# WJGiles/Dorknet

Measured on AMD Instinct MI355X. Metric: images/sec training step, ResNet-18-depsep 225x225 bs=256, 1/2/4/8 MI355X, higher is better.
Workload: dtype fp32; 1 GPU; ResNet-18-depsep 225x225 training step (fwd+loss+bwd+SGD-momentum), BASELINE config 3; global_batch=256, per_gpu_batch=256, parallelism=dp1, batch_norm=local

## Files before the change

dorknet_amd/csrc/pw_deep.hip:

```cpp
#include <stdlib.h>

#include <algorithm>
#include <atomic>

#include "dk_common.h"
#include "fold_tail.h"

#ifndef DK_PWD_EXP
#define DK_PWD_EXP 0
#endif

namespace dk {
namespace pwd {

constexpr int TR = 32;
constexpr int NW = 4;
constexpr int NB = 32 * NW;
constexpr int NT = 64 * NW;
typedef uint32_t u32x4 __attribute__((ext_vector_type(4)));
typedef uint32_t u32x2 __attribute__((ext_vector_type(2)));

template <int KR>
constexpr int fwd_wps() {
  return KR <= 64 ? 4 : KR <= 128 ? 3 : KR <= 256 ? 2 : 1;
}
template <int KR>
constexpr int dgrad_wps() {
  return KR <= 128 ? 2 : 1;
}

__device__ __forceinline__ uint32_t off4(int m, int ld, int c) { return ((uint32_t)m * ld + c) * 4u; }

__device__ __forceinline__ __amdgpu_buffer_rsrc_t tile_rsrc(const float* p, int ld, int tile, int nrows) {
  const int rows = nrows - tile * TR;
  return make_rsrc_v(p + (size_t)tile * TR * ld, rows > 0 ? (uint32_t)rows * ld * 4u : 0u);
}

constexpr int kAD = 4;

__device__ __forceinline__ int first_tile(int ntiles) {
  const int G = gridDim.x, r = ntiles % G, s = (r + 7) & ~7;
  return (int)((blockIdx.x + (unsigned)blockIdx.y * (unsigned)s) % (unsigned)G);
}
template <int KQ>
__device__ __forceinline__ void mfma_tile(const float* ap, const f32x4* bw, f32x16& acc) {
  constexpr int D = KQ < kAD ? KQ : kAD;
#pragma unroll
  for (int r = 0; r < 16; ++r) acc[r] = 0.f;
  f32x4 ab[D];
#pragma unroll
  for (int i = 0; i < D; ++i) ab[i] = ld4(ap + 8 * i);
#pragma unroll
  for (int q = 0; q < KQ; ++q) {
    const f32x4 av = ab[q % D];
    if (q + D < KQ) ab[q % D] = ld4(ap + 8 * (q + D));
    __builtin_amdgcn_sched_barrier(0);
#pragma unroll
    for (int e = 0; e < 4; ++e) acc = __builtin_amdgcn_mfma_f32_32x32x2f32(av[e], bw[q][e], acc, 0, 0, 0);
    __builtin_amdgcn_sched_barrier(0);
  }
}

__device__ __forceinline__ f32x4 cat4(f32x2 a, f32x2 b) { return f32x4{a[0], a[1], b[0], b[1]}; }
__device__ __forceinline__ f32x4 xhat4(f32x4 x, f32x4 m, f32x4 i) {
  return cat4((lo2(x) - lo2(m)) * lo2(i), (hi2(x) - hi2(m)) * hi2(i));
}
__device__ __forceinline__ f32x4 affine4(f32x4 xh, f32x4 g, f32x4 b) {
  return cat4(__builtin_elementwise_fma(lo2(g), lo2(xh), lo2(b)), __builtin_elementwise_fma(hi2(g), hi2(xh), hi2(b)));
}

struct FwdArgs {
  const float* x;
  const float* w;
  const float* bias;
  float* y;
  const float *im, *iis, *ig, *ib;
  int irelu;
  double* part;
  int M, N, H, W, OH, OW, sa;
  uint32_t xbytes;
  FoldTail ft;
  int nt;
};

__device__ __forceinline__ void partial_row(double ps, double pq, double* part, int N, int n0, const FoldTail& ft,
                                            float* scratch) {
  const int tid = threadIdx.x, lane = tid & 63, wave = tid >> 6, l32 = lane & 31, h = lane >> 5;
  double(*const red)[NB] = reinterpret_cast<double(*)[NB]>(scratch);
  ps += __shfl_xor(ps, 32, 64);
  pq += __shfl_xor(pq, 32, 64);
  __syncthreads();
  if (h == 0) {
    red[0][32 * wave + l32] = ps;
    red[1][32 * wave + l32] = pq;
  }
  __syncthreads();
  const int nc = N - n0 < NB ? N - n0 : NB;
  for (int i = tid; i < 2 * NB; i += NT) {
    const int which = i / NB, c = i - which * NB;
    if (c < nc) pub_store(part + ((size_t)blockIdx.x * 2 + which) * N + n0 + c, red[which][c]);
  }
  if (ft.part) {
    __syncthreads();
    fold_tail<NT>(ft, blockIdx.x, n0, nc, blockIdx.y, reinterpret_cast<double2*>(scratch));
  }
}

template <int KR, bool BN, bool STATS, bool STRIDED, bool HB>
__global__ __launch_bounds__(NT, fwd_wps<KR>()) void fwd_kernel(FwdArgs a) {
  constexpr int SK = KR + 4, KV = KR / 4, LV = TR * KV / NT, KQ = KR / 8;
  static_assert(KR % 32 == 0 && (SK / 4) % 2 == 1 && NT % KV == 0, "pwd::fwd_kernel shape");
  __shared__ __attribute__((aligned(16))) float As[2][TR * SK];
  static_assert(sizeof(double) * 2 * NT <= sizeof(float) * 2 * TR * SK, "fold scratch fits in the tiles");

  const int tid = threadIdx.x, lane = tid & 63, wave = tid >> 6;
  const int l32 = lane & 31, h = lane >> 5;
  const int n0 = blockIdx.y * NB, N = a.N;
  const int col = n0 + 32 * wave + l32;
  const float bias = HB ? a.bias[col] : 0.f;
  const bool irelu = a.irelu != 0;
  const int kv = tid % KV, r0 = tid / KV;
  f32x4 mu, is, ga, be;
  if constexpr (BN) {
    mu = ld4(a.im + 4 * kv);
    is = ld4(a.iis + 4 * kv);
    ga = ld4(a.ig + 4 * kv);
    be = ld4(a.ib + 4 * kv);
  }
  const __amdgpu_buffer_rsrc_t rx = make_rsrc_v(a.x, a.xbytes);
  const int ntiles = (a.M + TR - 1) / TR, G = gridDim.x;
  uint32_t lofs[LV], eofs[16];
#pragma unroll
  for (int j = 0; j < LV; ++j) lofs[j] = off4(r0 + j * (NT / KV), KR, 4 * kv);
#pragma unroll
  for (int r = 0; r < 16; ++r) eofs[r] = off4(4 * h + (r & 3) + 8 * (r >> 2), N, col);

  auto load_tile = [&](int tile, f32x4* st) {
    const __amdgpu_buffer_rsrc_t rt = tile_rsrc(a.x, KR, tile, a.M);
#pragma unroll
    for (int j = 0; j < LV; ++j) {
      if constexpr (STRIDED) {
        const int m = tile * TR + r0 + j * (NT / KV);
        const int ow = m % a.OW, q = m / a.OW, oh = q % a.OH, n = q / a.OH;
        const int row = (n * a.H + oh * a.sa) * a.W + ow * a.sa;
        st[j] = __builtin_bit_cast(f32x4, __builtin_amdgcn_raw_buffer_load_b128(rx, (int)off4(row, KR, 4 * kv), 0, 0));
      } else {
        st[j] = __builtin_bit_cast(f32x4, __builtin_amdgcn_raw_buffer_load_b128(rt, (int)lofs[j], 0, 0));
      }
    }
  };
  auto stage = [&](float* dst, const f32x4* st) {
    if (BN && irelu) {
#pragma unroll
      for (int j = 0; j < LV; ++j) {
        f32x4 v = st[j];
        if (!(DK_PWD_EXP & 2)) {
          v = affine4(xhat4(v, mu, is), ga, be);
#pragma unroll
          for (int e = 0; e < 4; ++e) v[e] = __builtin_fmaxf(v[e], 0.f);
        }
        st4(dst + (r0 + j * (NT / KV)) * SK + 4 * kv, v);
      }
    } else {
#pragma unroll
      for (int j = 0; j < LV; ++j) {
        f32x4 v = st[j];
        if constexpr (BN) v = affine4(xhat4(v, mu, is), ga, be);
        st4(dst + (r0 + j * (NT / KV)) * SK + 4 * kv, v);
      }
    }
  };

  int t = first_tile(ntiles);
  f32x4 bw[KQ];
  {
    f32x4 st[LV];
    load_tile(t, st);
#pragma unroll
    for (int q = 0; q < KQ; ++q)
      bw[q] = (DK_PWD_EXP & 8) ? f32x4{0.01f * q, 0.02f, 0.03f, (float)col} : ld4(a.w + (size_t)col * KR + 8 * q + 4 * h);
    stage(&As[0][0], st);
  }
  __syncthreads();
  double ps = 0.0, pq = 0.0;
  int buf = 0;
  for (; t < ntiles; t += G) {
    f32x4 nst[LV];
    load_tile(t + G, nst);
    const float* ap = &As[buf][0] + l32 * SK + 4 * h;
    f32x16 acc;
    mfma_tile<KQ>(ap, bw, acc);
    const int mb = t * TR + 4 * h;
    const __amdgpu_buffer_rsrc_t ry = tile_rsrc(a.y, N, t, a.M);
    if constexpr (HB) {
#pragma unroll
      for (int r = 0; r < 16; ++r) acc[r] += bias;
    }
#pragma unroll
    for (int r = 0; r < 16; ++r) {
      const float v = acc[r];
      if (!(DK_PWD_EXP & 1))
        bstore_nt(__builtin_bit_cast(uint32_t, v), ry, (int)eofs[r], 0, a.nt);
    }
    if constexpr (STATS) {
      if (t * TR + TR <= a.M) {
#pragma unroll
        for (int r = 0; r < 16; ++r) {
          const double d = (double)acc[r];
          ps += d;
          pq += d * d;
        }
      } else {
#pragma unroll
        for (int r = 0; r < 16; ++r) {
          const int dm = (r & 3) + 8 * (r >> 2);
          const double d = (mb + dm < a.M) ? (double)acc[r] : 0.0;
          ps += d;
          pq += d * d;
        }
      }
    }
    stage(&As[buf ^ 1][0], nst);
    __syncthreads();
    buf ^= 1;
  }
  if constexpr (STATS) partial_row(ps, pq, a.part, N, n0, a.ft, &As[0][0]);
}

struct DgradArgs {
  const float* g;
  const float* xo;
  float* dy_out;
  const float* w;
  float* dx;
  const float* res;
  const float* xi;
  const float *om, *ois, *og, *ob, *k12;
  int orelu;
  const float *im, *iis, *ig, *ib;
  int irelu;
  double* part;
  int M, N;
  FoldTail ft;
  int nt;
};

template <int KR, bool RES, bool PART, bool PLAIN = false>
__global__ __launch_bounds__(NT, dgrad_wps<KR>()) void dgrad_kernel(DgradArgs a) {
  constexpr int SK = KR + 4, KV = KR / 4, LV = TR * KV / NT, KQ = KR / 8;
  static_assert(KR % 32 == 0 && (SK / 4) % 2 == 1 && NT % KV == 0, "pwd::dgrad_kernel shape");
  __shared__ __attribute__((aligned(16))) float As[2][TR * SK];
  static_assert(sizeof(double) * 2 * NT <= sizeof(float) * 2 * TR * SK, "fold scratch fits in the tiles");

  const int tid = threadIdx.x, lane = tid & 63, wave = tid >> 6;
  const int l32 = lane & 31, h = lane >> 5;
  const int n0 = blockIdx.y * NB, N = a.N;
  const int col = n0 + 32 * wave + l32;
  const int kv = tid % KV, r0 = tid / KV;
  f32x4 mu = {}, is = {}, ga = {}, be = {}, k1 = {}, k2 = {}, f = {};
  if constexpr (!PLAIN) {
    mu = ld4(a.om + 4 * kv), is = ld4(a.ois + 4 * kv), ga = ld4(a.og + 4 * kv), be = ld4(a.ob + 4 * kv);
    k1 = ld4(a.k12 + 4 * kv), k2 = ld4(a.k12 + KR + 4 * kv);
#pragma unroll
    for (int e = 0; e < 4; ++e) f[e] = ga[e] * is[e];
  }
  const float pm = PART ? a.im[col] : 0.f, pis = PART ? a.iis[col] : 0.f, pga = PART ? a.ig[col] : 0.f,
              pbe = PART ? a.ib[col] : 0.f;
  const bool orelu = a.orelu != 0, irelu = a.irelu != 0;

  const bool writer = a.dy_out != nullptr && blockIdx.y == 0;
  const int ntiles = (a.M + TR - 1) / TR, G = gridDim.x;
  uint32_t lofs[LV], eofs[16];
#pragma unroll
  for (int j = 0; j < LV; ++j) lofs[j] = off4(r0 + j * (NT / KV), KR, 4 * kv);
#pragma unroll
  for (int r = 0; r < 16; ++r) eofs[r] = off4(4 * h + (r & 3) + 8 * (r >> 2), N, col);

  auto load_tile = [&](int tile, f32x4* sg, f32x4* sx) {
    const __amdgpu_buffer_rsrc_t rg = tile_rsrc(a.g, KR, tile, a.M), rx = tile_rsrc(a.xo, KR, tile, a.M);
#pragma unroll
    for (int j = 0; j < LV; ++j) {
      sg[j] = __builtin_bit_cast(f32x4, __builtin_amdgcn_raw_buffer_load_b128(rg, (int)lofs[j], 0, 0));
      if constexpr (!PLAIN)
        sx[j] = __builtin_bit_cast(f32x4, __builtin_amdgcn_raw_buffer_load_b128(rx, (int)lofs[j], 0, 0));
    }
  };
  auto stage = [&](int tile, float* dst, const f32x4* sg, const f32x4* sx) {
    const __amdgpu_buffer_rsrc_t rdy = tile_rsrc(writer ? a.dy_out : a.g, KR, tile, writer ? a.M : 0);
#pragma unroll
    for (int j = 0; j < LV; ++j) {
      const int r = r0 + j * (NT / KV);
      f32x4 v = sg[j];
      if constexpr (!PLAIN)
#pragma unroll
      for (int e = 0; e < 4; ++e) {
        const float xe = sx[j][e];
        float ge = sg[j][e];
        const bool kill = (!(bn_out(xe, mu[e], is[e], ga[e], be[e]) > 0.f)) & orelu;
        ge = kill ? 0.f : ge;
        v[e] = (DK_PWD_EXP & 2) ? ge + xe : bn_bwd_elem(xe, ge, mu[e], is[e], f[e], k1[e], k2[e]);
      }
      st4(dst + r * SK + 4 * kv, v);
      if constexpr (!PLAIN) bstore_nt(__builtin_bit_cast(u32x4, v), rdy, (int)lofs[j], 0, a.nt);
    }
  };

  int t = first_tile(ntiles);
  f32x4 bw[KQ];
  {
    f32x4 sg[LV], sx[LV];
    load_tile(t, sg, sx);
#pragma unroll
    for (int q = 0; q < KQ; ++q)
#pragma unroll
      for (int e = 0; e < 4; ++e) bw[q][e] = (DK_PWD_EXP & 8) ? 0.01f * q + e : a.w[(size_t)(8 * q + 4 * h + e) * N + col];
    stage(t, &As[0][0], sg, sx);
  }
  __syncthreads();
  double ps = 0.0, pq = 0.0;
  int buf = 0;
  for (; t < ntiles; t += G) {
    f32x4 ng[LV], nx[LV];
    load_tile(t + G, ng, nx);
    const int mb = t * TR + 4 * h;
    const __amdgpu_buffer_rsrc_t rxi = tile_rsrc(PART ? a.xi : a.g, N, t, PART ? a.M : 0);
    const __amdgpu_buffer_rsrc_t rr = tile_rsrc(RES ? a.res : a.g, N, t, RES ? a.M : 0);
    const __amdgpu_buffer_rsrc_t rdx = tile_rsrc(a.dx, N, t, a.M);
    float exi[16], ers[16];
#pragma unroll
    for (int r = 0; r < 16; ++r) {
      if constexpr (PART)
        exi[r] = __builtin_bit_cast(float, __builtin_amdgcn_raw_buffer_load_b32(rxi, (int)eofs[r], 0, 0));
      if constexpr (RES)
        ers[r] = __builtin_bit_cast(float, __builtin_amdgcn_raw_buffer_load_b32(rr, (int)eofs[r], 0, 0));
    }
    const float* ap = &As[buf][0] + l32 * SK + 4 * h;
    f32x16 acc;
    mfma_tile<KQ>(ap, bw, acc);
    if constexpr (RES) {
#pragma unroll
      for (int r = 0; r < 16; ++r) acc[r] += ers[r];
    }
#pragma unroll
    for (int r = 0; r < 16; ++r) {
      const float v = acc[r];
      if (!(DK_PWD_EXP & 1))
        bstore_nt(__builtin_bit_cast(uint32_t, v), rdx, (int)eofs[r], 0, a.nt);
    }
    if constexpr (PART) {
      const bool full = t * TR + TR <= a.M;
#pragma unroll
      for (int r = 0; r < 16; ++r) {
        const int dm = (r & 3) + 8 * (r >> 2);
        const float x = exi[r];
        const float xh = (x - pm) * pis;
        const bool kill = ((!(pga * xh + pbe > 0.f)) & irelu) | (!full && mb + dm >= a.M);
        const float gv = kill ? 0.f : acc[r];
        ps += (double)gv;
        pq += (double)gv * (double)xh;
      }
    }
    stage(t + G, &As[buf ^ 1][0], ng, nx);
    __syncthreads();
    buf ^= 1;
  }
  if constexpr (PART) partial_row(ps, pq, a.part, N, n0, a.ft, &As[0][0]);
}

constexpr int TR16 = 16;
constexpr int NW16 = 8;
constexpr int NT16 = 64 * NW16;

template <int KR>
struct K16 {
  static constexpr int RS = KR / 4 + 4;
  static constexpr int SK = 4 * RS + 4;
  static constexpr int KV = KR / 4;
  static constexpr int LV = TR16 * KV / NT16;
  static constexpr int NQ = KR / 16;
};

template <int NQ>
__device__ __forceinline__ void mfma16_tile(const float* ap, const f32x4* bw, f32x4& acc) {
  constexpr int D = 4;
  acc = f32x4{0.f, 0.f, 0.f, 0.f};
  f32x4 ab[D];
#pragma unroll
  for (int i = 0; i < D; ++i) ab[i] = ld4(ap + 4 * i);
#pragma unroll
  for (int q = 0; q < NQ; ++q) {
    const f32x4 av = ab[q % D];
    if (q + D < NQ) ab[q % D] = ld4(ap + 4 * (q + D));
    __builtin_amdgcn_sched_barrier(0);
#pragma unroll
    for (int u = 0; u < 4; ++u) acc = __builtin_amdgcn_mfma_f32_16x16x4f32(av[u], bw[q][u], acc, 0, 0, 0);
    __builtin_amdgcn_sched_barrier(0);
  }
}

template <int KR, bool RES, bool PART, bool PLAIN = false>
__global__ __launch_bounds__(NT16, 2) void dgrad16_kernel(DgradArgs a) {
  using L = K16<KR>;
  constexpr int SK = L::SK, RS = L::RS, KV = L::KV, LV = L::LV, NQ = L::NQ;
  static_assert(KR % 256 == 0 && (SK / 4) % 2 == 1 && NT16 % KV == 0 && LV >= 1, "pwd::dgrad16_kernel shape");
  __shared__ __attribute__((aligned(16))) float As[2][TR16 * SK];
  __shared__ __attribute__((aligned(16))) f32x4 bnt[7][KV];
  static_assert(sizeof(double) * 2 * NT16 <= sizeof(float) * 2 * TR16 * SK, "fold scratch fits in the tiles");

  const int tid = threadIdx.x, lane = tid & 63, wave = tid >> 6;
  const int c16 = lane & 15, kg = lane >> 4;
  const int n0 = blockIdx.y * NB, N = a.N;
  const int col = n0 + 16 * wave + c16;
  const int kvl = tid % KV, r0 = tid / KV;
  const int kv = (kvl & ~63) | ((kvl & 31) << 1) | ((kvl >> 5) & 1);
  if (!PLAIN && tid < KV) {
    const f32x4 ga = ld4(a.og + 4 * tid), is = ld4(a.ois + 4 * tid);
    bnt[0][tid] = ld4(a.om + 4 * tid);
    bnt[1][tid] = is;
    bnt[2][tid] = ga;
    bnt[3][tid] = ld4(a.ob + 4 * tid);
    bnt[4][tid] = ld4(a.k12 + 4 * tid);
    bnt[5][tid] = ld4(a.k12 + KR + 4 * tid);
    f32x4 f;
#pragma unroll
    for (int e = 0; e < 4; ++e) f[e] = ga[e] * is[e];
    bnt[6][tid] = f;
  }
  const float pm = PART ? a.im[col] : 0.f, pis = PART ? a.iis[col] : 0.f, pga = PART ? a.ig[col] : 0.f,
              pbe = PART ? a.ib[col] : 0.f;
  const bool orelu = a.orelu != 0, irelu = a.irelu != 0;
  const bool writer = a.dy_out != nullptr && blockIdx.y == 0;
  const int ntiles = (a.M + TR16 - 1) / TR16, G = gridDim.x;
  uint32_t lofs[LV];
#pragma unroll
  for (int j = 0; j < LV; ++j) lofs[j] = off4(r0 + j * (NT16 / KV), KR, 4 * kv);
  const uint32_t cbase = off4(4 * kg, N, col);
  const int sreg = (kv & 1) * RS + (kv & ~1);

  auto tile_rsrc16 = [&](const float* p, int ld, int tile, int nrows) {
    const int rows = nrows - tile * TR16;
    return make_rsrc_v(p + (size_t)tile * TR16 * ld, rows > 0 ? (uint32_t)rows * ld * 4u : 0u);
  };
  auto load_tile = [&](int tile, f32x4* sg, f32x4* sx) {
    const __amdgpu_buffer_rsrc_t rg = tile_rsrc16(a.g, KR, tile, a.M), rx = tile_rsrc16(a.xo, KR, tile, a.M);
#pragma unroll
    for (int j = 0; j < LV; ++j) {
      sg[j] = __builtin_bit_cast(f32x4, __builtin_amdgcn_raw_buffer_load_b128(rg, (int)lofs[j], 0, 0));
      if constexpr (!PLAIN)
        sx[j] = __builtin_bit_cast(f32x4, __builtin_amdgcn_raw_buffer_load_b128(rx, (int)lofs[j], 0, 0));
    }
  };
  auto stage = [&](int tile, float* dst, const f32x4* sg, const f32x4* sx) {
    const __amdgpu_buffer_rsrc_t rdy = tile_rsrc16(writer ? a.dy_out : a.g, KR, tile, writer ? a.M : 0);
#pragma unroll
    for (int j = 0; j < LV; ++j) {
      const int r = r0 + j * (NT16 / KV);
      f32x4 v = sg[j];
      if constexpr (!PLAIN) {
        const f32x4 mu = bnt[0][kv], is = bnt[1][kv], ga = bnt[2][kv], be = bnt[3][kv], k1 = bnt[4][kv],
                    k2 = bnt[5][kv], f = bnt[6][kv];
#pragma unroll
        for (int e = 0; e < 4; ++e) {
          const float xe = sx[j][e];
          float ge = sg[j][e];
          const bool kill = (!(bn_out(xe, mu[e], is[e], ga[e], be[e]) > 0.f)) & orelu;
          ge = kill ? 0.f : ge;
          v[e] = bn_bwd_elem(xe, ge, mu[e], is[e], f[e], k1[e], k2[e]);
        }
      }
      float* d = dst + r * SK + sreg;
      *reinterpret_cast<f32x2*>(d) = f32x2{v[0], v[2]};
      *reinterpret_cast<f32x2*>(d + 2 * RS) = f32x2{v[1], v[3]};
      if constexpr (!PLAIN) bstore_nt(__builtin_bit_cast(u32x4, v), rdy, (int)lofs[j], 0, a.nt);
    }
  };

  __syncthreads();
  int t = first_tile(ntiles);
  f32x4 bw[NQ];
  {
    f32x4 sg[LV], sx[LV];
    load_tile(t, sg, sx);
#pragma unroll
    for (int q = 0; q < NQ; ++q)
#pragma unroll
      for (int u = 0; u < 4; ++u) {
        const int i = 4 * q + u;
        const int k = 8 * (i >> 1) + 2 * (i & 1) + (kg >> 1) + 4 * (kg & 1);
        bw[q][u] = a.w[(size_t)k * N + col];
      }
    stage(t, &As[0][0], sg, sx);
  }
  __syncthreads();
  double ps = 0.0, pq = 0.0;
  int buf = 0;
  for (; t < ntiles; t += G) {
    f32x4 ng[LV], nx[LV];
    load_tile(t + G, ng, nx);
    const int mb = t * TR16 + 4 * kg;
    const __amdgpu_buffer_rsrc_t rxi = tile_rsrc16(PART ? a.xi : a.g, N, t, PART ? a.M : 0);
    const __amdgpu_buffer_rsrc_t rr = tile_rsrc16(RES ? a.res : a.g, N, t, RES ? a.M : 0);
    const __amdgpu_buffer_rsrc_t rdx = tile_rsrc16(a.dx, N, t, a.M);
    float exi[4], ers[4];
#pragma unroll
    for (int r = 0; r < 4; ++r) {
      if constexpr (PART)
        exi[r] = __builtin_bit_cast(float, __builtin_amdgcn_raw_buffer_load_b32(rxi, (int)cbase, r * N * 4, 0));
      if constexpr (RES)
        ers[r] = __builtin_bit_cast(float, __builtin_amdgcn_raw_buffer_load_b32(rr, (int)cbase, r * N * 4, 0));
    }
    f32x4 acc;
    mfma16_tile<NQ>(&As[buf][0] + c16 * SK + kg * RS, bw, acc);
    if constexpr (RES) {
#pragma unroll
      for (int r = 0; r < 4; ++r) acc[r] += ers[r];
    }
#pragma unroll
    for (int r = 0; r < 4; ++r) {
      const float v = acc[r];
      bstore_nt(__builtin_bit_cast(uint32_t, v), rdx, (int)cbase, r * N * 4, a.nt);
    }
    if constexpr (PART) {
      const bool full = t * TR16 + TR16 <= a.M;
#pragma unroll
      for (int r = 0; r < 4; ++r) {
        const float x = exi[r];
        const float xh = (x - pm) * pis;
        const bool kill = ((!(pga * xh + pbe > 0.f)) & irelu) | (!full && mb + r >= a.M);
        const float gv = kill ? 0.f : acc[r];
        ps += (double)gv;
        pq += (double)gv * (double)xh;
      }
    }
    stage(t + G, &As[buf ^ 1][0], ng, nx);
    __syncthreads();
    buf ^= 1;
  }
  if constexpr (PART) {
    double(*const red)[NB] = reinterpret_cast<double(*)[NB]>(&As[0][0]);
    ps += __shfl_xor(ps, 16, 64);
    pq += __shfl_xor(pq, 16, 64);
    ps += __shfl_xor(ps, 32, 64);
    pq += __shfl_xor(pq, 32, 64);
    __syncthreads();
    if (kg == 0) {
      red[0][16 * wave + c16] = ps;
      red[1][16 * wave + c16] = pq;
    }
    __syncthreads();
    for (int i = tid; i < 2 * NB; i += NT16) {
      const int which = i / NB, c = i - which * NB;
      pub_store(a.part + ((size_t)blockIdx.x * 2 + which) * N + n0 + c, red[which][c]);
    }
    if (a.ft.part) {
      __syncthreads();
      fold_tail<NT16>(a.ft, blockIdx.x, n0, NB, blockIdx.y, reinterpret_cast<double2*>(&As[0][0]));
    }
  }
}

struct BwdArgs {
  const float* g;
  const float* xo;
  const float* w;
  float* dx;
  const float* res;
  const float* xi;
  const float *om, *ois, *og, *ob, *k12;
  int orelu;
  const float *im, *iis, *ig, *ib;
  int irelu;
  double* part;
  float* wpart;
  int M, N;
  FoldTail ft;
  int nt;
};

template <int KR>
constexpr int bwd_wps() {
  return KR <= 128 ? 2 : 1;
}

template <int KR, bool RES, bool BNIN>
__global__ __launch_bounds__(NT, bwd_wps<KR>()) void bwd_kernel(BwdArgs a) {
  constexpr int SK = KR + 4, KV = KR / 4, LV = TR * KV / NT, KQ = KR / 8, NKT = KR / 32, NU = KR / 128;
  static_assert(KR % 128 == 0 && (SK / 4) % 2 == 1 && NT % KV == 0, "pwd::bwd_kernel shape");
  __shared__ __attribute__((aligned(16))) float As[2][TR * SK];
  __shared__ __attribute__((aligned(16))) f32x4 bnt[7][KV];
  static_assert(sizeof(double) * 2 * NT <= sizeof(float) * 2 * TR * SK, "fold scratch fits in the tiles");
  static_assert(32 * (NB + 4) <= 2 * TR * SK, "dW transpose tile fits in the tiles");

  const int tid = threadIdx.x, lane = tid & 63, wave = tid >> 6;
  const int l32 = lane & 31, h = lane >> 5;
  const int n0 = blockIdx.y * NB, N = a.N;
  const int col = n0 + 32 * wave + l32;
  const bool wact = n0 + 32 * wave < N;
  const int kv = tid % KV, r0 = tid / KV;
  if (tid < KV) {
    const f32x4 ga = ld4(a.og + 4 * tid), is = ld4(a.ois + 4 * tid);
    bnt[0][tid] = ld4(a.om + 4 * tid);
    bnt[1][tid] = is;
    bnt[2][tid] = ga;
    bnt[3][tid] = ld4(a.ob + 4 * tid);
    bnt[4][tid] = ld4(a.k12 + 4 * tid);
    bnt[5][tid] = ld4(a.k12 + KR + 4 * tid);
    f32x4 f;
#pragma unroll
    for (int e = 0; e < 4; ++e) f[e] = ga[e] * is[e];
    bnt[6][tid] = f;
  }
  __syncthreads();
  const float pm = BNIN && wact ? a.im[col] : 0.f, pis = BNIN && wact ? a.iis[col] : 0.f,
              pga = BNIN && wact ? a.ig[col] : 0.f, pbe = BNIN && wact ? a.ib[col] : 0.f;
  const bool orelu = a.orelu != 0, irelu = a.irelu != 0;

  const int ntiles = (a.M + TR - 1) / TR, G = gridDim.x;
  uint32_t lofs[LV];
#pragma unroll
  for (int j = 0; j < LV; ++j) lofs[j] = off4(r0 + j * (NT / KV), KR, 4 * kv);
  const uint32_t cbase = off4(4 * h, N, col);

  auto load_tile = [&](int tile, f32x4* sg, f32x4* sx) {
    const __amdgpu_buffer_rsrc_t rg = tile_rsrc(a.g, KR, tile, a.M), rx = tile_rsrc(a.xo, KR, tile, a.M);
#pragma unroll
    for (int j = 0; j < LV; ++j) {
      sg[j] = __builtin_bit_cast(f32x4, __builtin_amdgcn_raw_buffer_load_b128(rg, (int)lofs[j], 0, 0));
      sx[j] = __builtin_bit_cast(f32x4, __builtin_amdgcn_raw_buffer_load_b128(rx, (int)lofs[j], 0, 0));
    }
  };
  auto stage = [&](float* dst, const f32x4* sg, const f32x4* sx) {
    const f32x4 mu = bnt[0][kv], is = bnt[1][kv], ga = bnt[2][kv], be = bnt[3][kv], k1 = bnt[4][kv], k2 = bnt[5][kv],
                f = bnt[6][kv];
#pragma unroll
    for (int j = 0; j < LV; ++j) {
      const int r = r0 + j * (NT / KV);
      f32x4 v;
#pragma unroll
      for (int e = 0; e < 4; ++e) {
        const float xe = sx[j][e];
        float ge = sg[j][e];
        const bool kill = (!(bn_out(xe, mu[e], is[e], ga[e], be[e]) > 0.f)) & orelu;
        ge = kill ? 0.f : ge;
        v[e] = bn_bwd_elem(xe, ge, mu[e], is[e], f[e], k1[e], k2[e]);
      }
      st4(dst + r * SK + 4 * kv, v);
    }
  };

  int t = first_tile(ntiles);
  f32x4 bw[KQ];
  {
    f32x4 sg[LV], sx[LV];
    load_tile(t, sg, sx);
#pragma unroll
    for (int q = 0; q < KQ; ++q)
#pragma unroll
      for (int e = 0; e < 4; ++e) bw[q][e] = wact ? a.w[(size_t)(8 * q + 4 * h + e) * N + col] : 0.f;
    stage(&As[0][0], sg, sx);
  }
  __syncthreads();
  f32x16 dw[NKT];
#pragma unroll
  for (int i = 0; i < NKT; ++i)
#pragma unroll
    for (int r = 0; r < 16; ++r) dw[i][r] = 0.f;
  double ps = 0.0, pq = 0.0;
  int buf = 0;
  for (; t < ntiles; t += G) {
    f32x4 ng[LV], nx[LV];
    load_tile(t + G, ng, nx);
    const float* tile = &As[buf][0];
    if (wact) {
    const int mb = t * TR + 4 * h;
    const __amdgpu_buffer_rsrc_t rxi = tile_rsrc(a.xi, N, t, a.M);
    const __amdgpu_buffer_rsrc_t rr = tile_rsrc(RES ? a.res : a.xi, N, t, RES ? a.M : 0);
    const __amdgpu_buffer_rsrc_t rdx = tile_rsrc(a.dx, N, t, a.M);
    float ex[16], ers[16];
#pragma unroll
    for (int r = 0; r < 16; ++r) {
      const int ro = ((r & 3) + 8 * (r >> 2)) * N * 4;
      ex[r] = __builtin_bit_cast(float, __builtin_amdgcn_raw_buffer_load_b32(rxi, (int)cbase, ro, 0));
      if constexpr (RES) ers[r] = __builtin_bit_cast(float, __builtin_amdgcn_raw_buffer_load_b32(rr, (int)cbase, ro, 0));
    }
    f32x16 acc;
    mfma_tile<KQ>(tile + l32 * SK + 4 * h, bw, acc);
    if constexpr (RES) {
#pragma unroll
      for (int r = 0; r < 16; ++r) acc[r] += ers[r];
    }
#pragma unroll
    for (int r = 0; r < 16; ++r) {
      const float v = acc[r];
      bstore_nt(__builtin_bit_cast(uint32_t, v), rdx, (int)cbase, ((r & 3) + 8 * (r >> 2)) * N * 4, a.nt);
    }
    const bool full = t * TR + TR <= a.M;
    float yb[16];
#pragma unroll
    for (int r = 0; r < 16; ++r) {
      const int dm = (r & 3) + 8 * (r >> 2);
      const bool out = !full && mb + dm >= a.M;
      const float x = ex[r];
      if constexpr (BNIN) {
        const float xh = (x - pm) * pis;
        const float v = __builtin_fmaf(pga, xh, pbe);
        const bool dead = !(v > 0.f) & irelu;
        const float gv = (dead | out) ? 0.f : acc[r];
        ps += (double)gv;
        pq += (double)gv * (double)xh;
        yb[r] = (dead | out) ? 0.f : v;
      } else {
        yb[r] = out ? 0.f : x;
      }
    }
    {
      const float* bp = tile + (4 * h) * SK + 4 * l32;
      f32x4 bv[NU], nb[NU];
#pragma unroll
      for (int u = 0; u < NU; ++u) bv[u] = ld4(bp + 128 * u);
#pragma unroll
      for (int s = 0; s < 16; ++s) {
        if (s + 1 < 16) {
          const int pn = ((s + 1) & 3) + 8 * ((s + 1) >> 2);
#pragma unroll
          for (int u = 0; u < NU; ++u) nb[u] = ld4(bp + pn * SK + 128 * u);
        }
        __builtin_amdgcn_sched_barrier(0);
#pragma unroll
        for (int u = 0; u < NU; ++u)
#pragma unroll
          for (int e = 0; e < 4; ++e) dw[4 * u + e] = __builtin_amdgcn_mfma_f32_32x32x2f32(yb[s], bv[u][e], dw[4 * u + e], 0, 0, 0);
        __builtin_amdgcn_sched_barrier(0);
#pragma unroll
        for (int u = 0; u < NU; ++u) bv[u] = nb[u];
      }
    }
    }
    stage(&As[buf ^ 1][0], ng, nx);
    __syncthreads();
    buf ^= 1;
  }
  {
    constexpr int ST = NB + 4;
    float* T = &As[0][0];
    float* wp = a.wpart + (size_t)blockIdx.x * KR * N + n0;
#pragma unroll
    for (int kt = 0; kt < NKT; ++kt) {
      __syncthreads();
#pragma unroll
      for (int r = 0; r < 16; ++r) T[l32 * ST + 32 * wave + 4 * h + (r & 3) + 8 * (r >> 2)] = dw[kt][r];
      __syncthreads();
#pragma unroll
      for (int j = 0; j < 32 * NB / 4 / NT; ++j) {
        const int idx = tid + NT * j, i = idx / (NB / 4), c4 = idx % (NB / 4);
        const int k = 4 * i + (kt & 3) + 128 * (kt >> 2);
        if (n0 + 4 * c4 < N) st4(wp + (size_t)k * N + 4 * c4, ld4(T + i * ST + 4 * c4));
      }
    }
  }
  if constexpr (BNIN) partial_row(ps, pq, a.part, N, n0, a.ft, &As[0][0]);
}

template <int KR, bool RES, bool BNIN>
__global__ __launch_bounds__(NT16, 2) void bwd16_kernel(BwdArgs a) {
  using L = K16<KR>;
  constexpr int SK = L::SK, RS = L::RS, KV = L::KV, LV = L::LV, NQ = L::NQ, NKT = KR / 16;
  static_assert(KR % 256 == 0 && (SK / 4) % 2 == 1 && NT16 % KV == 0 && LV >= 1, "pwd::bwd16_kernel shape");
  __shared__ __attribute__((aligned(16))) float As[2][TR16 * SK];
  __shared__ __attribute__((aligned(16))) f32x4 bnt[7][KV];
  static_assert(sizeof(double) * 2 * NT16 <= sizeof(float) * 2 * TR16 * SK, "fold scratch fits in the tiles");

  const int tid = threadIdx.x, lane = tid & 63, wave = tid >> 6;
  const int c16 = lane & 15, kg = lane >> 4;
  const int n0 = blockIdx.y * NB, N = a.N;
  const int col = n0 + 16 * wave + c16;
  const int kvl = tid % KV, r0 = tid / KV;
  const int kv = (kvl & ~63) | ((kvl & 31) << 1) | ((kvl >> 5) & 1);
  if (tid < KV) {
    const f32x4 ga = ld4(a.og + 4 * tid), is = ld4(a.ois + 4 * tid);
    bnt[0][tid] = ld4(a.om + 4 * tid);
    bnt[1][tid] = is;
    bnt[2][tid] = ga;
    bnt[3][tid] = ld4(a.ob + 4 * tid);
    bnt[4][tid] = ld4(a.k12 + 4 * tid);
    bnt[5][tid] = ld4(a.k12 + KR + 4 * tid);
    f32x4 f;
#pragma unroll
    for (int e = 0; e < 4; ++e) f[e] = ga[e] * is[e];
    bnt[6][tid] = f;
  }
  const float pm = BNIN ? a.im[col] : 0.f, pis = BNIN ? a.iis[col] : 0.f, pga = BNIN ? a.ig[col] : 0.f,
              pbe = BNIN ? a.ib[col] : 0.f;
  const bool orelu = a.orelu != 0, irelu = a.irelu != 0;
  const int ntiles = (a.M + TR16 - 1) / TR16, G = gridDim.x;
  uint32_t lofs[LV];
#pragma unroll
  for (int j = 0; j < LV; ++j) lofs[j] = off4(r0 + j * (NT16 / KV), KR, 4 * kv);
  const uint32_t cbase = off4(4 * kg, N, col);
  const int sreg = (kv & 1) * RS + (kv & ~1);
  const int r8 = c16 & 7;
  const int doff = ((((r8 & 1) << 1) | ((r8 >> 2) & 1)) * RS) + 2 * (c16 >> 3) + ((r8 >> 1) & 1);

  auto tile_rsrc16 = [&](const float* p, int ld, int tile, int nrows) {
    const int rows = nrows - tile * TR16;
    return make_rsrc_v(p + (size_t)tile * TR16 * ld, rows > 0 ? (uint32_t)rows * ld * 4u : 0u);
  };
  auto load_tile = [&](int tile, f32x4* sg, f32x4* sx) {
    const __amdgpu_buffer_rsrc_t rg = tile_rsrc16(a.g, KR, tile, a.M), rx = tile_rsrc16(a.xo, KR, tile, a.M);
#pragma unroll
    for (int j = 0; j < LV; ++j) {
      sg[j] = __builtin_bit_cast(f32x4, __builtin_amdgcn_raw_buffer_load_b128(rg, (int)lofs[j], 0, 0));
      sx[j] = __builtin_bit_cast(f32x4, __builtin_amdgcn_raw_buffer_load_b128(rx, (int)lofs[j], 0, 0));
    }
  };
  auto stage = [&](float* dst, const f32x4* sg, const f32x4* sx) {
    const f32x4 mu = bnt[0][kv], is = bnt[1][kv], ga = bnt[2][kv], be = bnt[3][kv], k1 = bnt[4][kv], k2 = bnt[5][kv],
                f = bnt[6][kv];
#pragma unroll
    for (int j = 0; j < LV; ++j) {
      const int r = r0 + j * (NT16 / KV);
      f32x4 v;
#pragma unroll
      for (int e = 0; e < 4; ++e) {
        const float xe = sx[j][e];
        float ge = sg[j][e];
        const bool kill = (!(bn_out(xe, mu[e], is[e], ga[e], be[e]) > 0.f)) & orelu;
        ge = kill ? 0.f : ge;
        v[e] = bn_bwd_elem(xe, ge, mu[e], is[e], f[e], k1[e], k2[e]);
      }
      float* d = dst + r * SK + sreg;
      *reinterpret_cast<f32x2*>(d) = f32x2{v[0], v[2]};
      *reinterpret_cast<f32x2*>(d + 2 * RS) = f32x2{v[1], v[3]};
    }
  };

  __syncthreads();
  int t = first_tile(ntiles);
  f32x4 bw[NQ];
  {
    f32x4 sg[LV], sx[LV];
    load_tile(t, sg, sx);
#pragma unroll
    for (int q = 0; q < NQ; ++q)
#pragma unroll
      for (int u = 0; u < 4; ++u) {
        const int i = 4 * q + u;
        const int k = 8 * (i >> 1) + 2 * (i & 1) + (kg >> 1) + 4 * (kg & 1);
        bw[q][u] = a.w[(size_t)k * N + col];
      }
    stage(&As[0][0], sg, sx);
  }
  __syncthreads();
  f32x4 dw[NKT];
#pragma unroll
  for (int i = 0; i < NKT; ++i) dw[i] = f32x4{0.f, 0.f, 0.f, 0.f};
  double ps = 0.0, pq = 0.0;
  int buf = 0;
  for (; t < ntiles; t += G) {
    f32x4 ng[LV], nx[LV];
    load_tile(t + G, ng, nx);
    const int mb = t * TR16 + 4 * kg;
    const __amdgpu_buffer_rsrc_t rxi = tile_rsrc16(a.xi, N, t, a.M);
    const __amdgpu_buffer_rsrc_t rr = tile_rsrc16(RES ? a.res : a.xi, N, t, RES ? a.M : 0);
    const __amdgpu_buffer_rsrc_t rdx = tile_rsrc16(a.dx, N, t, a.M);
    float ex[4], ers[4];
#pragma unroll
    for (int r = 0; r < 4; ++r) {
      ex[r] = __builtin_bit_cast(float, __builtin_amdgcn_raw_buffer_load_b32(rxi, (int)cbase, r * N * 4, 0));
      if constexpr (RES)
        ers[r] = __builtin_bit_cast(float, __builtin_amdgcn_raw_buffer_load_b32(rr, (int)cbase, r * N * 4, 0));
    }
    const float* tile = &As[buf][0];
    f32x4 acc;
    mfma16_tile<NQ>(tile + c16 * SK + kg * RS, bw, acc);
    if constexpr (RES) {
#pragma unroll
      for (int r = 0; r < 4; ++r) acc[r] += ers[r];
    }
#pragma unroll
    for (int r = 0; r < 4; ++r) {
      const float v = acc[r];
      bstore_nt(__builtin_bit_cast(uint32_t, v), rdx, (int)cbase, r * N * 4, a.nt);
    }
    const bool full = t * TR16 + TR16 <= a.M;
    float yb[4];
#pragma unroll
    for (int r = 0; r < 4; ++r) {
      const bool out = !full && mb + r >= a.M;
      const float x = ex[r];
      if constexpr (BNIN) {
        const float xh = (x - pm) * pis;
        const float v = __builtin_fmaf(pga, xh, pbe);
        const bool dead = !(v > 0.f) & irelu;
        const float gv = (dead | out) ? 0.f : acc[r];
        ps += (double)gv;
        pq += (double)gv * (double)xh;
        yb[r] = (dead | out) ? 0.f : v;
      } else {
        yb[r] = out ? 0.f : x;
      }
    }
    {
      const float* bp = tile + (4 * kg) * SK + doff;
#pragma unroll
      for (int r = 0; r < 4; ++r) {
        float bv[NKT];
#pragma unroll
        for (int kt = 0; kt < NKT; ++kt) bv[kt] = bp[r * SK + 4 * kt];
#pragma unroll
        for (int kt = 0; kt < NKT; ++kt) dw[kt] = __builtin_amdgcn_mfma_f32_16x16x4f32(yb[r], bv[kt], dw[kt], 0, 0, 0);
      }
    }
    stage(&As[buf ^ 1][0], ng, nx);
    __syncthreads();
    buf ^= 1;
  }
  {
    float* wp = a.wpart + (size_t)blockIdx.x * KR * N + n0 + 16 * wave + 4 * kg;
#pragma unroll
    for (int kt = 0; kt < NKT; ++kt) st4(wp + (size_t)(16 * kt + c16) * N, dw[kt]);
  }
  if constexpr (BNIN) {
    double(*const red)[NB] = reinterpret_cast<double(*)[NB]>(&As[0][0]);
    ps += __shfl_xor(ps, 16, 64);
    pq += __shfl_xor(pq, 16, 64);
    ps += __shfl_xor(ps, 32, 64);
    pq += __shfl_xor(pq, 32, 64);
    __syncthreads();
    if (kg == 0) {
      red[0][16 * wave + c16] = ps;
      red[1][16 * wave + c16] = pq;
    }
    __syncthreads();
    for (int i = tid; i < 2 * NB; i += NT16) {
      const int which = i / NB, c = i - which * NB;
      pub_store(a.part + ((size_t)blockIdx.x * 2 + which) * N + n0 + c, red[which][c]);
    }
    if (a.ft.part) {
      __syncthreads();
      fold_tail<NT16>(a.ft, blockIdx.x, n0, NB, blockIdx.y, reinterpret_cast<double2*>(&As[0][0]));
    }
  }
}

#define DK_PWD_KR(X) X(64) X(128) X(256) X(512)
#define DK_PWD_KR_DGRAD(X) X(64) X(128) X(256)

static int occupancy(const void* fn, int nt = NT) {
  int v = 0;
  if (hipOccupancyMaxActiveBlocksPerMultiprocessor(&v, fn, nt, 0) != hipSuccess || v < 1) v = 1;
  return v;
}

template <int KR>
static int fwd_occ() {
  static const int occ = [] {
#define DK_F(B_, S_, T_) reinterpret_cast<const void*>(&fwd_kernel<KR, B_, S_, T_, false>), \
                         reinterpret_cast<const void*>(&fwd_kernel<KR, B_, S_, T_, true>)
    const void* fs[] = {DK_F(true, true, false), DK_F(true, false, false), DK_F(false, true, false),
                        DK_F(false, false, false), DK_F(true, true, true), DK_F(true, false, true),
                        DK_F(false, true, true), DK_F(false, false, true)};
#undef DK_F
    int o = 1 << 20;
    for (const void* f : fs) o = std::min(o, occupancy(f));
    return o;
  }();
  return occ;
}
template <int KR>
static int dgrad_occ() {
  static const int occ = [] {
    const void* fs[] = {reinterpret_cast<const void*>(&dgrad_kernel<KR, true, true>),
                        reinterpret_cast<const void*>(&dgrad_kernel<KR, true, false>),
                        reinterpret_cast<const void*>(&dgrad_kernel<KR, false, true>),
                        reinterpret_cast<const void*>(&dgrad_kernel<KR, false, false>)};
    int o = 1 << 20;
    for (const void* f : fs) o = std::min(o, occupancy(f));
    return o;
  }();
  return occ;
}

template <int KR>
static int dgrad16_occ() {
  static const int occ = [] {
    const void* fs[] = {reinterpret_cast<const void*>(&dgrad16_kernel<KR, true, true>),
                        reinterpret_cast<const void*>(&dgrad16_kernel<KR, true, false>),
                        reinterpret_cast<const void*>(&dgrad16_kernel<KR, false, true>),
                        reinterpret_cast<const void*>(&dgrad16_kernel<KR, false, false>)};
    int o = 1 << 20;
    for (const void* f : fs) o = std::min(o, occupancy(f, NT16));
    return o;
  }();
  return occ;
}

template <int KR>
static int bwd16_occ() {
  static const int occ = [] {
    const void* fs[] = {reinterpret_cast<const void*>(&bwd16_kernel<KR, true, true>),
                        reinterpret_cast<const void*>(&bwd16_kernel<KR, true, false>),
                        reinterpret_cast<const void*>(&bwd16_kernel<KR, false, true>),
                        reinterpret_cast<const void*>(&bwd16_kernel<KR, false, false>)};
    int o = 1 << 20;
    for (const void* f : fs) o = std::min(o, occupancy(f, NT16));
    return o;
  }();
  return occ;
}

template <int KR>
static int bwd_occ() {
  static const int occ = [] {
    const void* fs[] = {reinterpret_cast<const void*>(&bwd_kernel<KR, true, true>),
                        reinterpret_cast<const void*>(&bwd_kernel<KR, true, false>),
                        reinterpret_cast<const void*>(&bwd_kernel<KR, false, true>),
                        reinterpret_cast<const void*>(&bwd_kernel<KR, false, false>)};
    int o = 1 << 20;
    for (const void* f : fs) o = std::min(o, occupancy(f));
    return o;
  }();
  return occ;
}

static int grid_x(int M, int N, int occ, int tr = TR) {
  const int ntiles = (M + tr - 1) / tr;
  const int groups = N < NB ? 1 : N / NB;
  int slots = occ * 256 / groups;
  if (slots < 1) slots = 1;
  int gx = std::min(ntiles, slots);
  const int g8 = gx / 8 * 8;
  if (g8 >= 8 && (ntiles + g8 - 1) / g8 == (ntiles + gx - 1) / gx) gx = g8;
  return gx;
}

}

static bool pwd_enabled() { return knob(kKnobPwDeep) == 1 && pw_stream_enabled(); }

static bool pwd_kr(int KR) { return KR == 64 || KR == 128 || KR == 256 || KR == 512; }

bool pw_deep_fwd_ok(int K, int C, int M, size_t xbytes) {
  if (!pwd_enabled() || M <= 0 || (K < 128 && C < 128) || !pwd_kr(C) || K % pwd::NB) return false;
  return xbytes < ((size_t)1 << 31) && (size_t)M * K * 4 < ((size_t)1 << 31);
}
bool pw_deep_dgrad_ok(int K, int C, int M) {
  if (!pwd_enabled() || M <= 0 || (K < 128 && C < 128) || !pwd_kr(K) || C % pwd::NB) return false;
  return (size_t)M * (K > C ? K : C) * 4 < ((size_t)1 << 31);
}

int pw_deep_fwd_rows(int M, int K, int C) {
#define DK_ROWS(kr) \
  if (C == kr) return pwd::grid_x(M, K, pwd::fwd_occ<kr>());
  DK_PWD_KR(DK_ROWS)
#undef DK_ROWS
  return 0;
}
int pw_deep_fwd_slices(int M, int K, int C) { return K / pwd::NB; }
static bool pwd_dgrad16(int K) { return K == 512; }

int pw_deep_dgrad_rows(int M, int K, int C) {
  if (pwd_dgrad16(K)) return pwd::grid_x(M, C, pwd::dgrad16_occ<512>(), pwd::TR16);
#define DK_ROWS(kr) \
  if (K == kr) return pwd::grid_x(M, C, pwd::dgrad_occ<kr>());
  DK_PWD_KR_DGRAD(DK_ROWS)
#undef DK_ROWS
  return 0;
}
int pw_deep_dgrad_slices(int M, int K, int C) { return C / pwd::NB; }

int pw_deep_fwd(const float* x, int N, int H, int W, int stride, int OH, int OW, const float* w, int K, int C,
                const float* bias, float* y, const float* im, const float* iis, const float* ig, const float* ib,
                int irelu, double* part, hipStream_t st, const FoldTail* ft) {
  const int M = N * OH * OW;
  const bool strided = stride != 1 || H != OH || W != OW;
  pwd::FwdArgs a{x, w, bias, y, im, iis, ig, ib, irelu, part, M, K, H, W, OH, OW, stride,
                 (uint32_t)((size_t)N * H * W * C * 4)};
  if (ft && part) a.ft = *ft;
  a.nt = nt_stores(kNtPwd);
  const dim3 grid(pw_deep_fwd_rows(M, K, C), K / pwd::NB);
  if (grid.x == 0) return DK_ERR_ARGS;
#define DK_L(kr, B_, S_, T_)                                                                          \
  do {                                                                                                \
    if (bias)                                                                                         \
      hipLaunchKernelGGL((pwd::fwd_kernel<kr, B_, S_, T_, true>), grid, dim3(pwd::NT), 0, st, a);     \
    else                                                                                              \
      hipLaunchKernelGGL((pwd::fwd_kernel<kr, B_, S_, T_, false>), grid, dim3(pwd::NT), 0, st, a);    \
  } while (0)
#define DK_FWD(kr)                    \
  if (C == kr) {                      \
    if (strided) {                    \
      if (im && part)                 \
        DK_L(kr, true, true, true);   \
      else if (im)                    \
        DK_L(kr, true, false, true);  \
      else if (part)                  \
        DK_L(kr, false, true, true);  \
      else                            \
        DK_L(kr, false, false, true); \
    } else if (im && part)            \
      DK_L(kr, true, true, false);    \
    else if (im)                      \
      DK_L(kr, true, false, false);   \
    else if (part)                    \
      DK_L(kr, false, true, false);   \
    else                              \
      DK_L(kr, false, false, false);  \
    return launch_status();           \
  }
  DK_PWD_KR(DK_FWD)
#undef DK_FWD
#undef DK_L
  return DK_ERR_ARGS;
}

int pw_deep_dgrad_bnbwd(const float* g, const float* bn_x, int M, int K, int C, const float* om, const float* ois,
                        const float* og, const float* ob, int orelu, const float* k12, float* dy_out, const float* w,
                        float* dx, const float* res, const float* x, const float* im, const float* iis,
                        const float* ig, const float* ib, int irelu, double* part, hipStream_t st,
                        const FoldTail* ft) {
  pwd::DgradArgs a{g, bn_x, dy_out, w, dx, res, x, om, ois, og, ob, k12, orelu, im, iis, ig, ib, irelu, part, M, C};
  if (ft && part) a.ft = *ft;
  a.nt = nt_stores(kNtPwd);
  const dim3 grid(pw_deep_dgrad_rows(M, K, C), C / pwd::NB);
  if (grid.x == 0) return DK_ERR_ARGS;
  if (pwd_dgrad16(K)) {
#define DK_L16(R_, P_) hipLaunchKernelGGL((pwd::dgrad16_kernel<512, R_, P_>), grid, dim3(pwd::NT16), 0, st, a)
    if (res && x)
      DK_L16(true, true);
    else if (res)
      DK_L16(true, false);
    else if (x)
      DK_L16(false, true);
    else
      DK_L16(false, false);
#undef DK_L16
    return launch_status();
  }
#define DK_L(kr, R_, P_) hipLaunchKernelGGL((pwd::dgrad_kernel<kr, R_, P_>), grid, dim3(pwd::NT), 0, st, a)
#define DK_DG(kr)             \
  if (K == kr) {              \
    if (res && x)             \
      DK_L(kr, true, true);   \
    else if (res)             \
      DK_L(kr, true, false);  \
    else if (x)               \
      DK_L(kr, false, true);  \
    else                      \
      DK_L(kr, false, false); \
    return launch_status();   \
  }
  DK_PWD_KR_DGRAD(DK_DG)
#undef DK_DG
#undef DK_L
  return DK_ERR_ARGS;
}

int pw_deep_dgrad_plain(const float* dy, int M, int K, int C, const float* w, float* dx, hipStream_t st) {
  pwd::DgradArgs a{dy, nullptr, nullptr, w, dx, nullptr, nullptr, nullptr, nullptr, nullptr, nullptr, nullptr, 0,
                   nullptr, nullptr, nullptr, nullptr, 0, nullptr, M, C};
  a.nt = nt_stores(kNtPwd);
  const dim3 grid(pw_deep_dgrad_rows(M, K, C), C / pwd::NB);
  if (grid.x == 0) return DK_ERR_ARGS;
  if (pwd_dgrad16(K)) {
    hipLaunchKernelGGL((pwd::dgrad16_kernel<512, false, false, true>), grid, dim3(pwd::NT16), 0, st, a);
    return launch_status();
  }
#define DK_DG(kr)                                                                                           \
  if (K == kr) {                                                                                            \
    hipLaunchKernelGGL((pwd::dgrad_kernel<kr, false, false, true>), grid, dim3(pwd::NT), 0, st, a);         \
    return launch_status();                                                                                 \
  }
  DK_PWD_KR_DGRAD(DK_DG)
#undef DK_DG
  return DK_ERR_ARGS;
}

static bool pwd_bwd_enabled() { return knob(kKnobPwDeepBwd) == 1 && pwd_enabled(); }
bool pw_deep_bwd_ok(int K, int C, int M) {
  if (!pwd_bwd_enabled() || M <= 0 || (K != 128 && K != 256) || (C % pwd::NB && !(K == 128 && C == 64)))
    return false;
  return (size_t)M * (K > C ? K : C) * 4 < ((size_t)1 << 31);
}
static bool pwd_bwd16(int K) { return K == 256; }

int pw_deep_bwd_rows(int M, int K, int C) {
  if (pwd_bwd16(K)) return pwd::grid_x(M, C, pwd::bwd16_occ<256>(), pwd::TR16);
  if (K == 128) return pwd::grid_x(M, C, pwd::bwd_occ<128>());
  return 0;
}
int pw_deep_bwd_slices(int M, int K, int C) { return C < pwd::NB ? 1 : C / pwd::NB; }

int pw_deep_bwd_bnbwd(const float* g, const float* bn_x, int M, int K, int C, const float* om, const float* ois,
                      const float* og, const float* ob, int orelu, const float* k12, const float* w, float* dx,
                      const float* res, const float* x, const float* im, const float* iis, const float* ig,
                      const float* ib, int irelu, double* part, float* wpart, hipStream_t st, const FoldTail* ft) {
  if ((im != nullptr) != (part != nullptr)) return DK_ERR_ARGS;
  pwd::BwdArgs a{g, bn_x, w, dx, res, x, om, ois, og, ob, k12, orelu, im, iis, ig, ib, irelu, part, wpart, M, C};
  if (ft && part) a.ft = *ft;
  a.nt = nt_stores(kNtPwd);
  const dim3 grid(pw_deep_bwd_rows(M, K, C), pw_deep_bwd_slices(M, K, C));
  if (grid.x == 0) return DK_ERR_ARGS;
  if (pwd_bwd16(K)) {
#define DK_L16(kr, R_, B_) hipLaunchKernelGGL((pwd::bwd16_kernel<kr, R_, B_>), grid, dim3(pwd::NT16), 0, st, a)
#define DK_B16(kr)             \
  if (K == kr) {               \
    if (res && im)             \
      DK_L16(kr, true, true);  \
    else if (res)              \
      DK_L16(kr, true, false); \
    else if (im)               \
      DK_L16(kr, false, true); \
    else                       \
      DK_L16(kr, false, false); \
    return launch_status();    \
  }
    DK_B16(256)
#undef DK_B16
#undef DK_L16
  }
#define DK_L(kr, R_, B_) hipLaunchKernelGGL((pwd::bwd_kernel<kr, R_, B_>), grid, dim3(pwd::NT), 0, st, a)
#define DK_BW(kr)             \
  if (K == kr) {              \
    if (res && im)            \
      DK_L(kr, true, true);   \
    else if (res)             \
      DK_L(kr, true, false);  \
    else if (im)              \
      DK_L(kr, false, true);  \
    else                      \
      DK_L(kr, false, false); \
    return launch_status();   \
  }
  DK_BW(128)
#undef DK_BW
#undef DK_L
  return DK_ERR_ARGS;
}


}
```

Measured before the change: 33310 images/s.

## Add specialized pointwise backward kernel for K=128, C=64 processing tile pairs

Adds a dedicated fused backward kernel for the K=128, C=64 pointwise layer. The generic kernel uses a 128-column block, which leaves half of it idle when C is 64. The new kernel has each pair of waves cover the 64 columns and work on one of two 32-row tiles, so each block handles 64 rows per step. The two waves' dW partials are summed through shared memory before they are written. This is meant to recover the lanes wasted on the narrow layer, at the cost of more code, extra register pressure and an extra shared-memory reduction pass.

```diff
diff --git a/dorknet_amd/csrc/pw_deep.hip b/dorknet_amd/csrc/pw_deep.hip
--- a/dorknet_amd/csrc/pw_deep.hip
+++ b/dorknet_amd/csrc/pw_deep.hip
@@ -761,6 +761,207 @@
   if constexpr (BNIN) partial_row(ps, pq, a.part, N, n0, a.ft, &As[0][0]);
 }
 
+constexpr int TP = 2 * TR;
+
+template <bool RES, bool BNIN>
+__global__ __launch_bounds__(NT, 2) void bwd64_kernel(BwdArgs a) {
+  constexpr int KR = 128, N = 64, SK = KR + 4, KV = KR / 4, LV = TR * KV / NT, KQ = KR / 8, NKT = KR / 32;
+  static_assert((SK / 4) % 2 == 1 && NT % KV == 0, "pwd::bwd64_kernel shape");
+  __shared__ __attribute__((aligned(16))) float As[2][TP * SK];
+  __shared__ __attribute__((aligned(16))) f32x4 bnt[7][KV];
+  static_assert(sizeof(double) * 2 * NT <= sizeof(float) * 2 * TP * SK, "fold scratch fits in the tiles");
+  static_assert(32 * (N + 4) <= 2 * TP * SK, "dW transpose tile fits in the tiles");
+
+  const int tid = threadIdx.x, lane = tid & 63, wave = tid >> 6;
+  const int l32 = lane & 31, h = lane >> 5;
+  const int wp = __builtin_amdgcn_readfirstlane(wave >> 1);
+  const int col = 32 * (wave & 1) + l32;
+  const int kv = tid % KV, r0 = tid / KV;
+  if (tid < KV) {
+    const f32x4 ga = ld4(a.og + 4 * tid), is = ld4(a.ois + 4 * tid);
+    bnt[0][tid] = ld4(a.om + 4 * tid);
+    bnt[1][tid] = is;
+    bnt[2][tid] = ga;
+    bnt[3][tid] = ld4(a.ob + 4 * tid);
+    bnt[4][tid] = ld4(a.k12 + 4 * tid);
+    bnt[5][tid] = ld4(a.k12 + KR + 4 * tid);
+    f32x4 f;
+#pragma unroll
+    for (int e = 0; e < 4; ++e) f[e] = ga[e] * is[e];
+    bnt[6][tid] = f;
+  }
+  __syncthreads();
+  const float pm = BNIN ? a.im[col] : 0.f, pis = BNIN ? a.iis[col] : 0.f, pga = BNIN ? a.ig[col] : 0.f,
+              pbe = BNIN ? a.ib[col] : 0.f;
+  const bool orelu = a.orelu != 0, irelu = a.irelu != 0;
+
+  const int npairs = (a.M + TP - 1) / TP, G = gridDim.x;
+  const uint32_t lbase = off4(r0, KR, 4 * kv);
+  const uint32_t cbase = off4(4 * h, N, col);
+
+  auto load_tile = [&](int tile, f32x4* sg, f32x4* sx) {
+    const __amdgpu_buffer_rsrc_t rg = tile_rsrc(a.g, KR, tile, a.M), rx = tile_rsrc(a.xo, KR, tile, a.M);
+#pragma unroll
+    for (int j = 0; j < LV; ++j) {
+      const int ro = j * (NT / KV) * KR * 4;
+      sg[j] = __builtin_bit_cast(f32x4, __builtin_amdgcn_raw_buffer_load_b128(rg, (int)lbase, ro, 0));
+      sx[j] = __builtin_bit_cast(f32x4, __builtin_amdgcn_raw_buffer_load_b128(rx, (int)lbase, ro, 0));
+    }
+  };
+  auto stage = [&](float* dst, const f32x4* sg, const f32x4* sx) {
+    const f32x4 mu = bnt[0][kv], is = bnt[1][kv], ga = bnt[2][kv], be = bnt[3][kv], k1 = bnt[4][kv], k2 = bnt[5][kv],
+                f = bnt[6][kv];
+#pragma unroll
+    for (int j = 0; j < LV; ++j) {
+      const int r = r0 + j * (NT / KV);
+      f32x4 v;
+#pragma unroll
+      for (int e = 0; e < 4; ++e) {
+        const float xe = sx[j][e];
+        float ge = sg[j][e];
+        const bool kill = (!(bn_out(xe, mu[e], is[e], ga[e], be[e]) > 0.f)) & orelu;
+        ge = kill ? 0.f : ge;
+        v[e] = bn_bwd_elem(xe, ge, mu[e], is[e], f[e], k1[e], k2[e]);
+      }
+      st4(dst + r * SK + 4 * kv, v);
+    }
+  };
+
+  int p = blockIdx.x;
+  f32x4 bw[KQ];
+  {
+    f32x4 sg[LV], sx[LV], sg1[LV], sx1[LV];
+    load_tile(2 * p, sg, sx);
+    load_tile(2 * p + 1, sg1, sx1);
+#pragma unroll
+    for (int q = 0; q < KQ; ++q)
+#pragma unroll
+      for (int e = 0; e < 4; ++e) bw[q][e] = a.w[(size_t)(8 * q + 4 * h + e) * N + col];
+    stage(&As[0][0], sg, sx);
+    stage(&As[0][TR * SK], sg1, sx1);
+  }
+  __syncthreads();
+  f32x16 dw[NKT];
+#pragma unroll
+  for (int i = 0; i < NKT; ++i)
+#pragma unroll
+    for (int r = 0; r < 16; ++r) dw[i][r] = 0.f;
+  double ps = 0.0, pq = 0.0;
+  int buf = 0;
+  for (; p < npairs; p += G) {
+    f32x4 ng[LV], nx[LV];
+    load_tile(2 * (p + G), ng, nx);
+    const int t = 2 * p + wp;
+    const float* tile = &As[buf][wp * TR * SK];
+    const int mb = t * TR + 4 * h;
+    const __amdgpu_buffer_rsrc_t rxi = tile_rsrc(a.xi, N, t, a.M);
+    const __amdgpu_buffer_rsrc_t rr = tile_rsrc(RES ? a.res : a.xi, N, t, RES ? a.M : 0);
+    const __amdgpu_buffer_rsrc_t rdx = tile_rsrc(a.dx, N, t, a.M);
+    float ex[16], ers[16];
+#pragma unroll
+    for (int r = 0; r < 16; ++r) {
+      const int ro = ((r & 3) + 8 * (r >> 2)) * N * 4;
+      ex[r] = __builtin_bit_cast(float, __builtin_amdgcn_raw_buffer_load_b32(rxi, (int)cbase, ro, 0));
+      if constexpr (RES) ers[r] = __builtin_bit_cast(float, __builtin_amdgcn_raw_buffer_load_b32(rr, (int)cbase, ro, 0));
+    }
+    f32x16 acc;
+    mfma_tile<KQ>(tile + l32 * SK + 4 * h, bw, acc);
+    if constexpr (RES) {
+#pragma unroll
+      for (int r = 0; r < 16; ++r) acc[r] += ers[r];
+    }
+#pragma unroll
+    for (int r = 0; r < 16; ++r) {
+      const float v = acc[r];
+      bstore_nt(__builtin_bit_cast(uint32_t, v), rdx, (int)cbase, ((r & 3) + 8 * (r >> 2)) * N * 4, a.nt);
+    }
+    const bool full = t * TR + TR <= a.M;
+    float yb[16];
+#pragma unroll
+    for (int r = 0; r < 16; ++r) {
+      const int dm = (r & 3) + 8 * (r >> 2);
+      const bool out = !full && mb + dm >= a.M;
+      const float x = ex[r];
+      if constexpr (BNIN) {
+        const float xh = (x - pm) * pis;
+        const float v = __builtin_fmaf(pga, xh, pbe);
+        const bool dead = !(v > 0.f) & irelu;
+        const float gv = (dead | out) ? 0.f : acc[r];
+        ps += (double)gv;
+        pq += (double)gv * (double)xh;
+        yb[r] = (dead | out) ? 0.f : v;
+      } else {
+        yb[r] = out ? 0.f : x;
+      }
+    }
+    stage(&As[buf ^ 1][0], ng, nx);
+    load_tile(2 * (p + G) + 1, ng, nx);
+    {
+      const float* bp = tile + (4 * h) * SK + 4 * l32;
+      f32x4 bv = ld4(bp), nb;
+#pragma unroll
+      for (int s = 0; s < 16; ++s) {
+        if (s + 1 < 16) {
+          const int pn = ((s + 1) & 3) + 8 * ((s + 1) >> 2);
+          nb = ld4(bp + pn * SK);
+        }
+        __builtin_amdgcn_sched_barrier(0);
+#pragma unroll
+        for (int e = 0; e < 4; ++e) dw[e] = __builtin_amdgcn_mfma_f32_32x32x2f32(yb[s], bv[e], dw[e], 0, 0, 0);
+        __builtin_amdgcn_sched_barrier(0);
+        bv = nb;
+      }
+    }
+    stage(&As[buf ^ 1][TR * SK], ng, nx);
+    __syncthreads();
+    buf ^= 1;
+  }
+  {
+    constexpr int ST = N + 4;
+    float* T = &As[0][0];
+    float* wpr = a.wpart + (size_t)blockIdx.x * KR * N;
+    float* tl = T + l32 * ST + 32 * (wave & 1) + 4 * h;
+#pragma unroll
+    for (int kt = 0; kt < NKT; ++kt) {
+      __syncthreads();
+      if (wp == 1) {
+#pragma unroll
+        for (int r = 0; r < 16; ++r) tl[(r & 3) + 8 * (r >> 2)] = dw[kt][r];
+      }
+      __syncthreads();
+      if (wp == 0) {
+#pragma unroll
+        for (int r = 0; r < 16; ++r) tl[(r & 3) + 8 * (r >> 2)] = dw[kt][r] + tl[(r & 3) + 8 * (r >> 2)];
+      }
+      __syncthreads();
+#pragma unroll
+      for (int j = 0; j < 32 * N / 4 / NT; ++j) {
+        const int idx = tid + NT * j, i = idx / (N / 4), c4 = idx % (N / 4);
+        st4(wpr + (size_t)(4 * i + kt) * N + 4 * c4, ld4(T + i * ST + 4 * c4));
+      }
+    }
+  }
+  if constexpr (BNIN) {
+    double(*const red)[2][N] = reinterpret_cast<double(*)[2][N]>(&As[0][0]);
+    ps += __shfl_xor(ps, 32, 64);
+    pq += __shfl_xor(pq, 32, 64);
+    __syncthreads();
+    if (h == 0) {
+      red[wp][0][col] = ps;
+      red[wp][1][col] = pq;
+    }
+    __syncthreads();
+    if (tid < 2 * N) {
+      const int which = tid / N, c = tid - which * N;
+      pub_store(a.part + ((size_t)blockIdx.x * 2 + which) * N + c, red[0][which][c] + red[1][which][c]);
+    }
+    if (a.ft.part) {
+      __syncthreads();
+      fold_tail<NT>(a.ft, blockIdx.x, 0, N, 0, reinterpret_cast<double2*>(&As[0][0]));
+    }
+  }
+}
+
 template <int KR, bool RES, bool BNIN>
 __global__ __launch_bounds__(NT16, 2) void bwd16_kernel(BwdArgs a) {
   using L = K16<KR>;
@@ -1004,6 +1205,19 @@
                         reinterpret_cast<const void*>(&bwd16_kernel<KR, false, false>)};
     int o = 1 << 20;
     for (const void* f : fs) o = std::min(o, occupancy(f, NT16));
+    return o;
+  }();
+  return occ;
+}
+
+static int bwd64_occ() {
+  static const int occ = [] {
+    const void* fs[] = {reinterpret_cast<const void*>(&bwd64_kernel<true, true>),
+                        reinterpret_cast<const void*>(&bwd64_kernel<true, false>),
+                        reinterpret_cast<const void*>(&bwd64_kernel<false, true>),
+                        reinterpret_cast<const void*>(&bwd64_kernel<false, false>)};
+    int o = 1 << 20;
+    for (const void* f : fs) o = std::min(o, occupancy(f));
     return o;
   }();
   return occ;
@@ -1183,9 +1397,11 @@
   return (size_t)M * (K > C ? K : C) * 4 < ((size_t)1 << 31);
 }
 static bool pwd_bwd16(int K) { return K == 256; }
+static bool pwd_bwd64(int K, int C) { return K == 128 && C == 64; }
 
 int pw_deep_bwd_rows(int M, int K, int C) {
   if (pwd_bwd16(K)) return pwd::grid_x(M, C, pwd::bwd16_occ<256>(), pwd::TR16);
+  if (pwd_bwd64(K, C)) return pwd::grid_x(M, C, pwd::bwd64_occ(), pwd::TP);
   if (K == 128) return pwd::grid_x(M, C, pwd::bwd_occ<128>());
   return 0;
 }
@@ -1219,6 +1435,19 @@
 #undef DK_B16
 #undef DK_L16
   }
+  if (pwd_bwd64(K, C)) {
+#define DK_L64(R_, B_) hipLaunchKernelGGL((pwd::bwd64_kernel<R_, B_>), grid, dim3(pwd::NT), 0, st, a)
+    if (res && im)
+      DK_L64(true, true);
+    else if (res)
+      DK_L64(true, false);
+    else if (im)
+      DK_L64(false, true);
+    else
+      DK_L64(false, false);
+#undef DK_L64
+    return launch_status();
+  }
 #define DK_L(kr, R_, B_) hipLaunchKernelGGL((pwd::bwd_kernel<kr, R_, B_>), grid, dim3(pwd::NT), 0, st, a)
 #define DK_BW(kr)             \
   if (K == kr) {              \
```

Result: no change. 33500 images/s (median of 6 runs) (+0.6%).
